# christoskokas/gtsam-vSLAM

Measured on AMD Instinct MI355X. Metric: frames/sec (extract+match+localBA), 1500 feat stereo 752x480, higher is better.
Workload: dtype u8/i32 (extract, match) + f64 (pose LM, local BA)

## Files before the change

### gtsam-vslam_amd/csrc/extract_kernels.hip

```cpp
#include "extract_kernels.hpp"
#include "../../include/vslam_orb_pattern.h"
#include <cfloat>

namespace vslam {

__constant__ __attribute__((aligned(16))) signed char c_pattern[1024];

void upload_pattern() {
    (void)hipMemcpyToSymbol(HIP_SYMBOL(c_pattern), VSLAM_ORB_PATTERN, 1024);
}

__device__ __forceinline__ int resize_hsum(unsigned d0, unsigned d1, unsigned d2, bool upper, unsigned sel, int coef) {
    typedef short s16x2 __attribute__((ext_vector_type(2)));
    const unsigned taps = __builtin_amdgcn_perm(upper ? d2 : d1, upper ? d1 : d0, sel);
    return __builtin_amdgcn_sdot2(__builtin_bit_cast(s16x2, taps), __builtin_bit_cast(s16x2, coef), 0, false);
}

__global__ __launch_bounds__(256) void k_resize(uint8_t* __restrict__ pyr, PyrDesc P, int level,
                                                const int2* __restrict__ xtab,
                                                const int2* __restrict__ ytab) {
    const int img = blockIdx.z;
    const uint8_t* __restrict__ S = pyr + (size_t)img * P.imgStride + P.off[level - 1];
    uint8_t* __restrict__ D = pyr + (size_t)img * P.imgStride + P.off[level];
    const int sp = P.pitch[level - 1], dp = P.pitch[level];
    const int dw = P.w[level], dh = P.h[level], sh = P.h[level - 1];
    const int x0 = (blockIdx.x * 64 + threadIdx.x) * 4;
    const int y = blockIdx.y * 4 + __builtin_amdgcn_readfirstlane(threadIdx.y);
    if (y >= dh || x0 >= dw) return;
    const int2 yt = ytab[y];
    int sy0 = yt.x, sy1 = yt.x + 1;
    sy0 = sy0 < 0 ? 0 : (sy0 < sh ? sy0 : sh - 1);
    sy1 = sy1 < 0 ? 0 : (sy1 < sh ? sy1 : sh - 1);
    const int b0 = (short)(yt.y & 0xffff), b1 = (short)(yt.y >> 16);
    const uint8_t* r0 = S + (size_t)sy0 * sp;
    const uint8_t* r1 = S + (size_t)sy1 * sp;
    const int4 ta = *(const int4*)(xtab + x0), tb = *(const int4*)(xtab + x0 + 2);
    const int xs[4] = {ta.x, ta.z, tb.x, tb.z}, xc[4] = {ta.y, ta.w, tb.y, tb.w};
    const int base = (xs[0] & 0xffff) & ~3;
    int o0[4], o1[4];
    bool fits = true;
#pragma unroll
    for (int i = 0; i < 4; i++) {
        o0[i] = (xs[i] & 0xffff) - base;
        o1[i] = (int)((unsigned)xs[i] >> 16) - base;
        fits = fits && (unsigned)o0[i] < 12u && (unsigned)o1[i] < 12u && (unsigned)(o1[i] - o0[i]) <= 1u;
    }
    unsigned o = 0;
    if (fits) {
        const unsigned a0 = *(const unsigned*)(r0 + base), a1 = *(const unsigned*)(r0 + base + 4), a2 = *(const unsigned*)(r0 + base + 8);
        const unsigned c0 = *(const unsigned*)(r1 + base), c1 = *(const unsigned*)(r1 + base + 4), c2 = *(const unsigned*)(r1 + base + 8);
#pragma unroll
        for (int i = 0; i < 4; i++) {
            const bool upper = o1[i] > 7 || o0[i] > 7;
            const int sh4 = upper ? 4 : 0;
            const unsigned sel = (unsigned)(o0[i] - sh4) | ((unsigned)(o1[i] - sh4) << 16) | 0x0c000c00u;
            const int h0 = resize_hsum(a0, a1, a2, upper, sel, xc[i]);
            const int h1 = resize_hsum(c0, c1, c2, upper, sel, xc[i]);
            const unsigned v = (unsigned)((((b0 * (h0 >> 4)) >> 16) + ((b1 * (h1 >> 4)) >> 16) + 2) >> 2) & 0xffu;
            o |= (x0 + i < dw ? v : 0u) << (8 * i);
        }
    } else {
        uint8_t* op = (uint8_t*)&o;
#pragma unroll
        for (int i = 0; i < 4; i++) {
            if (x0 + i < dw) {
                const int sx = xs[i] & 0xffff, sx1 = (int)((unsigned)xs[i] >> 16);
                const int c0 = (short)(xc[i] & 0xffff), c1 = (short)(xc[i] >> 16);
                const int h0 = r0[sx] * c0 + r0[sx1] * c1;
                const int h1 = r1[sx] * c0 + r1[sx1] * c1;
                op[i] = (uint8_t)((((b0 * (h0 >> 4)) >> 16) + ((b1 * (h1 >> 4)) >> 16) + 2) >> 2);
            }
        }
    }
    *(unsigned*)(D + (size_t)y * dp + x0) = o;
}

__global__ __launch_bounds__(256) void k_load_images(const uint8_t* const* __restrict__ src, int stride, uint8_t* __restrict__ pyr,
                                                     PyrDesc P) {
    const int img = blockIdx.z;
    const uint8_t* __restrict__ S = src[img];
    if (!S) return;
    uint8_t* __restrict__ D = pyr + (size_t)img * P.imgStride + P.off[0];
    const int w = P.w[0], h = P.h[0], dp = P.pitch[0];
    const int y = blockIdx.y * 4 + threadIdx.y;
    const int x0 = (blockIdx.x * 64 + threadIdx.x) * 16;
    if (y >= h || x0 >= w) return;
    const uint8_t* sp = S + (size_t)y * stride + x0;
    uint8_t* dq = D + (size_t)y * dp + x0;
    if (x0 + 16 <= w && ((((uintptr_t)sp) | ((uintptr_t)dq)) & 15) == 0) *(uint4*)dq = *(const uint4*)sp;
    else for (int i = 0; i < 16 && x0 + i < w; i++) dq[i] = sp[i];
}
void launch_load_images(hipStream_t s, const uint8_t* const* dSrc, int stride, uint8_t* pyr, const PyrDesc& P, int nimg) {
    hipLaunchKernelGGL(k_load_images, dim3((P.w[0] + 1023) / 1024, (P.h[0] + 3) / 4, nimg), dim3(64, 4), 0, s, dSrc, stride, pyr, P);
}

template <int CN>
__global__ __launch_bounds__(256) void k_load_images_color(const uint8_t* const* __restrict__ src, int stride,
                                                           uint8_t* __restrict__ pyr, PyrDesc P) {
    const int img = blockIdx.z;
    const uint8_t* __restrict__ S = src[img];
    if (!S) return;
    uint8_t* __restrict__ D = pyr + (size_t)img * P.imgStride + P.off[0];
    const int w = P.w[0], h = P.h[0], dp = P.pitch[0];
    const int y = blockIdx.y * 4 + threadIdx.y;
    const int x0 = (blockIdx.x * 64 + threadIdx.x) * 16;
    if (y >= h || x0 >= w) return;
    const uint8_t* sp = S + (size_t)y * stride + (size_t)x0 * CN;
    uint8_t* dq = D + (size_t)y * dp + x0;
    if (x0 + 16 <= w && ((((uintptr_t)sp) | ((uintptr_t)dq)) & 15) == 0) {
        unsigned wd[4 * CN];
#pragma unroll
        for (int k = 0; k < CN; k++) {
            const uint4 v = ((const uint4*)sp)[k];
            wd[4 * k] = v.x; wd[4 * k + 1] = v.y; wd[4 * k + 2] = v.z; wd[4 * k + 3] = v.w;
        }
        unsigned o[4] = {0u, 0u, 0u, 0u};
#pragma unroll
        for (int p = 0; p < 16; p++) {
            const int bi = p * CN;
            const int b = (wd[bi >> 2] >> (8 * (bi & 3))) & 0xff;
            const int g = (wd[(bi + 1) >> 2] >> (8 * ((bi + 1) & 3))) & 0xff;
            const int r = (wd[(bi + 2) >> 2] >> (8 * ((bi + 2) & 3))) & 0xff;
            o[p >> 2] |= (unsigned)bgr_to_gray(b, g, r) << (8 * (p & 3));
        }
        *(uint4*)dq = make_uint4(o[0], o[1], o[2], o[3]);
    } else {
        for (int i = 0; i < 16 && x0 + i < w; i++)
            dq[i] = (uint8_t)bgr_to_gray(sp[i * CN], sp[i * CN + 1], sp[i * CN + 2]);
    }
}
void launch_load_images_color(hipStream_t s, const uint8_t* const* dSrc, int stride, int channels, uint8_t* pyr, const PyrDesc& P,
                              int nimg) {
    const dim3 grid((P.w[0] + 1023) / 1024, (P.h[0] + 3) / 4, nimg), block(64, 4);
    if (channels == 3) hipLaunchKernelGGL(k_load_images_color<3>, grid, block, 0, s, dSrc, stride, pyr, P);
    else hipLaunchKernelGGL(k_load_images_color<4>, grid, block, 0, s, dSrc, stride, pyr, P);
}

#define VS_GLOBAL __attribute__((address_space(1)))
typedef const VS_GLOBAL uint8_t* gbytes_t;
struct __attribute__((packed)) Packed2 { unsigned short v; };
struct __attribute__((packed)) Packed4 { unsigned v; };
// ... 447 lines not shown
                 uint32_t* cellSlots, int* cellCount, int maxThr, int minThr, int nimg) {
    dim3 grid((F.cellBase[P.nLevels] + 3) / 4, xcd_image_rows(nimg));
    const size_t lds = (size_t)4 * ((size_t)F.tileRows * F.tilePitch * 2 + 2 * (FQ_MASK + 1) * 2 + FQ3_CAP * 2);
    int listCap = FQ3_CAP;
    if (const char* e = getenv("VSLAM_FAST_LIST_CAP")) listCap = std::max(0, std::min(FQ3_CAP, atoi(e)));
    hipLaunchKernelGGL(k_fast, grid, dim3(256), lds, s, pyr, P, F, cellSlots, cellCount, maxThr, minThr, listCap, nimg);
}

#ifdef VSLAM_FAST_CHECK
int fast_check_failures(hipStream_t s) {
    int n = 0;
    if (hipStreamSynchronize(s) != hipSuccess) return -1;
    if (hipMemcpyFromSymbol(&n, HIP_SYMBOL(g_fastCheckFail), sizeof(int)) != hipSuccess) return -1;
    return n;
}
#endif

__global__ __launch_bounds__(1024) void k_gather(const uint32_t* __restrict__ cellSlots,
                                                 const int* __restrict__ cellCount, FastDesc F,
                                                 int nLevels, int* __restrict__ cellOff,
                                                 uint32_t* __restrict__ cand, int candCap,
                                                 int* __restrict__ levelCount) {
    extern __shared__ int soff[];
    __shared__ int wtot[16];
    __shared__ int s_run;
    const int img = blockIdx.x, tid = threadIdx.x, lane = tid & 63, wave = tid >> 6;
    const int nCells = F.cellBase[nLevels];
    const int* cnt = cellCount + (size_t)img * nCells;
    if (tid == 0) s_run = 0;
    __syncthreads();
    for (int base = 0; base < nCells; base += 1024) {
        const int i = base + tid;
        const int v = i < nCells ? cnt[i] : 0;
        int incl = v;
#pragma unroll
        for (int d = 1; d < 64; d <<= 1) {
            const int n = __shfl_up(incl, d);
            if (lane >= d) incl += n;
        }
        if (lane == 63) wtot[wave] = incl;
        __syncthreads();
        int woff = 0;
        for (int k = 0; k < wave; k++) woff += wtot[k];
        const int run = s_run;
        if (i < nCells) soff[i] = run + woff + incl - v;
        __syncthreads();
        if (tid == 1023) s_run = run + woff + incl;
        __syncthreads();
    }
    const int total = s_run;
    if (tid == 0) soff[nCells] = total;
    __syncthreads();
    if (blockIdx.y == 0) {
        int* off = cellOff + (size_t)img * (nCells + 1);
        for (int i = tid; i <= nCells; i += 1024) off[i] = soff[i];
        if (tid < nLevels) levelCount[img * (MAX_LEVELS + 1) + tid] = soff[F.cellBase[tid + 1]] - soff[F.cellBase[tid]];
        if (tid == 0) levelCount[img * (MAX_LEVELS + 1) + MAX_LEVELS] = total;
    }
    uint32_t* out = cand + (size_t)img * candCap;
    const int lim = min(total, candCap);
    for (int j = blockIdx.y * 1024 + tid; j < lim; j += gridDim.y * 1024) {
        int lo = 0, hi = nCells;
        while (lo < hi) {
            const int mid = (lo + hi) >> 1;
            if (soff[mid + 1] > j) hi = mid; else lo = mid + 1;
        }
        out[j] = cellSlots[((size_t)img * nCells + lo) * F.cellCap + (j - soff[lo])];
    }
}

void launch_gather(hipStream_t s, const uint32_t* cellSlots, const int* cellCount, const FastDesc& F,
                   int nLevels, int* cellOff, uint32_t* cand, int candCap, int* levelCount, int nimg) {
    const int nCells = F.cellBase[nLevels];
    hipLaunchKernelGGL(k_gather, dim3(nimg, 8), dim3(1024), (size_t)(nCells + 1) * sizeof(int), s, cellSlots, cellCount, F, nLevels,
                       cellOff, cand, candCap, levelCount);
}

__device__ __forceinline__ int reflect101(int p, int len) {
    if (len == 1) return 0;
    while (p < 0 || p >= len) p = p < 0 ? -p : 2 * len - 2 - p;
    return p;
}

__global__ __launch_bounds__(256) void k_blur(const uint8_t* __restrict__ pyr,
                                              uint8_t* __restrict__ blur, PyrDesc P, BlurDesc B) {
    const int img = blockIdx.y;
    int level = 0;
    const int t = blockIdx.x;
    while (level + 1 < P.nLevels && t >= B.tileBase[level + 1]) level++;
    const int lt = t - B.tileBase[level];
    const int tyb = lt / B.tilesX[level], txb = lt - tyb * B.tilesX[level];
    const int w = P.w[level], h = P.h[level], pitch = P.pitch[level];
    const uint8_t* __restrict__ S = pyr + (size_t)img * P.imgStride + P.off[level];
    uint8_t* __restrict__ D = blur + (size_t)img * P.imgStride + P.off[level];
    const int x = txb * BLUR_TW + (threadIdx.x & 63) * 4;
    const int yb = tyb * BLUR_TH + __builtin_amdgcn_readfirstlane(threadIdx.x >> 6) * BLUR_RPT;
    if (yb >= h || x >= w) return;
    const unsigned tA = (unsigned)B.taps[0] | ((unsigned)B.taps[1] << 8) | ((unsigned)B.taps[2] << 16) | ((unsigned)B.taps[3] << 24);
    const unsigned tB = (unsigned)B.taps[4] | ((unsigned)B.taps[5] << 8) | ((unsigned)B.taps[6] << 16);
    const int t0 = B.taps[0], t1 = B.taps[1], t2 = B.taps[2], t3 = B.taps[3];
    const int m = w - x;
    unsigned s1 = 0x07060504u;
    unsigned sA = 0x03020100u, sB = 0x07060504u;
    if (m == 1) s1 = 0x01020304u;
    else if (m == 2) { s1 = 0x03040504u; sA = 0x00000002u; sB = 0x07060500u; }
    else if (m == 3) { s1 = 0x05060504u; sA = 0x00000304u; sB = 0x07060100u; }
    else if (m == 4) { sA = 0x00040506u; sB = 0x07020100u; }
    else if (m == 5) { sA = 0x05060700u; sB = 0x03020104u; }
    else if (m == 6) sB = 0x07040504u;
    const bool leftEdge = x == 0;
    const unsigned xo0 = leftEdge ? 0u : (unsigned)(x - 4), xo1 = (unsigned)x;
    unsigned hb[7][4];
#pragma unroll
    for (int rr = 0; rr < BLUR_RPT + 6; rr++) {
        int sy = yb + rr - 3;
        sy = sy < 0 ? -sy : sy;
        sy = sy >= h ? 2 * h - 2 - sy : sy;
        sy = sy < 0 ? 0 : sy;
        const uint8_t* row = S + (size_t)sy * pitch;
        unsigned d0 = *(const unsigned*)(row + xo0);
        const uint2 d12 = *(const uint2*)(row + xo1);
        unsigned d1 = d12.x, d2 = d12.y;
        {
            const unsigned mir = __builtin_amdgcn_perm(d2, d1, 0x01020304u);
            const unsigned tmp = __builtin_amdgcn_perm(d1, d0, sA);
            const unsigned n1 = __builtin_amdgcn_perm(d1, d0, s1);
            d2 = __builtin_amdgcn_perm(d2, tmp, sB);
            d1 = n1;
            d0 = leftEdge ? mir : d0;
        }
        unsigned nh[4];
        nh[0] = __builtin_amdgcn_udot4(__builtin_amdgcn_alignbyte(d1, d0, 1), tA, __builtin_amdgcn_udot4(__builtin_amdgcn_alignbyte(d2, d1, 1), tB, 0u, false), false);
        nh[1] = __builtin_amdgcn_udot4(__builtin_amdgcn_alignbyte(d1, d0, 2), tA, __builtin_amdgcn_udot4(__builtin_amdgcn_alignbyte(d2, d1, 2), tB, 0u, false), false);
        nh[2] = __builtin_amdgcn_udot4(__builtin_amdgcn_alignbyte(d1, d0, 3), tA, __builtin_amdgcn_udot4(__builtin_amdgcn_alignbyte(d2, d1, 3), tB, 0u, false), false);
        nh[3] = __builtin_amdgcn_udot4(d1, tA, __builtin_amdgcn_udot4(d2, tB, 0u, false), false);
#pragma unroll
        for (int i = 0; i < 4; i++) {
#pragma unroll
            for (int k = 0; k < 6; k++) hb[k][i] = hb[k + 1][i];
            hb[6][i] = nh[i] & 0xffffu;
        }
        if (rr >= 6) {
            const int y = yb + rr - 6;
            if (y < h) {
                unsigned o = 0;
#pragma unroll
                for (int i = 0; i < 4; i++) {
                    const unsigned acc = (unsigned)t0 * (hb[0][i] + hb[6][i]) + (unsigned)t1 * (hb[1][i] + hb[5][i]) +
                                         (unsigned)t2 * (hb[2][i] + hb[4][i]) + (unsigned)t3 * hb[3][i];
                    o |= ((acc + 32768u) >> 16) << (8 * i);
                }
                uint8_t* dq = D + (size_t)y * pitch + x;
                if (x + 4 <= w) *(unsigned*)dq = o;
                else for (int i = 0; i < 4 && x + i < w; i++) dq[i] = (uint8_t)(o >> (8 * i));
            }
        }
    }
}

void launch_blur(hipStream_t s, const uint8_t* pyr, uint8_t* blur, const PyrDesc& P,
                 const BlurDesc& B, int nimg) {
    hipLaunchKernelGGL(k_blur, dim3(B.tileBase[P.nLevels], nimg), dim3(256), 0, s, pyr, blur, P, B);
}

__device__ __forceinline__ float fast_atan2_deg(float y, float x) {
    const float scale = (float)(180 / 3.1415926535897932384626433832795);
    const float p1 = 0.9997878412794807f * scale;
    const float p3 = -0.3258083974640975f * scale;
    const float p5 = 0.1555786518463281f * scale;
    const float p7 = -0.04432655554792128f * scale;
    const float ax = fabsf(x), ay = fabsf(y);
    float a, c, c2;
    if (ax >= ay) {
        c = ay / (ax + (float)DBL_EPSILON);
        c2 = c * c;
        a = (((p7 * c2 + p5) * c2 + p3) * c2 + p1) * c;
    } else {
        c = ax / (ay + (float)DBL_EPSILON);
        c2 = c * c;
        a = 90.f - (((p7 * c2 + p5) * c2 + p3) * c2 + p1) * c;
    }
    if (x < 0) a = 180.f - a;
    if (y < 0) a = 360.f - a;
    return a;
}

__device__ __forceinline__ void sincos_deg_range(float xf, float& s_out, float& c_out) {
    const double x = (double)xf;
    const double kd = rint(x * 6.36619772367581382433e-01);
    const int k = (int)kd;
    double r = fma(-kd, 1.57079632673412561417e+00, x);
    r = fma(-kd, 6.07710050650619224932e-11, r);
    const double z = r * r;
    double ps = fma(z, 1.58969099521155010221e-10, -2.50507602534068634195e-08);
    ps = fma(z, ps, 2.75573137070700676789e-06);
    ps = fma(z, ps, -1.98412698298579493134e-04);
    ps = fma(z, ps, 8.33333333332248946124e-03);
    const double sn = fma(z * r, fma(z, ps, -1.66666666666666324348e-01), r);
    double pc = fma(z, -1.13596475577881948265e-11, 2.08757232129817482790e-09);
    pc = fma(z, pc, -2.75573143513906633035e-07);
    pc = fma(z, pc, 2.48015872894767294178e-05);
    pc = fma(z, pc, -1.38888888888741095749e-03);
    pc = fma(z, pc, 4.16666666666666019037e-02);
    const double cs = 1.0 - fma(0.5, z, -(z * (z * pc)));
    const double sq = (k & 1) ? cs : sn, cq = (k & 1) ? sn : cs;
    s_out = (float)((k & 2) ? -sq : sq);
    c_out = (float)(((k + 1) & 2) ? -cq : cq);
}

constexpr int OD_MROWS = 31, OD_MDW = 9;
constexpr int OD_ROWS = 39, OD_DW = 11;
__global__ __launch_bounds__(256) void k_orient_desc(
    const uint8_t* __restrict__ pyr, const uint8_t* __restrict__ blur, PyrDesc P, LevelTables T,
    const uint32_t* __restrict__ kept, const int* __restrict__ keptOff, int keptCap,
    DiscRows R, vslam_keypoint* __restrict__ kps,
    uint8_t* __restrict__ desc, int outCap, int nimg) {
    const int lane = threadIdx.x & 63;
    const int wave = __builtin_amdgcn_readfirstlane(threadIdx.x >> 6);
    int chunk, img;
    if (!xcd_image_block(nimg, chunk, img)) return;
    const int g = chunk * 4 + wave;
    const int* koff = keptOff + img * (MAX_LEVELS + 1);
    const int total = koff[P.nLevels];
    if (g >= total || g >= outCap) return;
    const int4 pat4 = *(const int4*)(c_pattern + 16 * lane);
    int level = 0;
    while (level + 1 < P.nLevels && g >= koff[level + 1]) level++;
    const uint32_t pk = kept[(size_t)img * keptCap + g];
    const int x = cand_x(pk), y = cand_y(pk), score = cand_s(pk);
    const int pitch = P.pitch[level];
    const size_t lvlOff = (size_t)img * P.imgStride + P.off[level];
    __shared__ unsigned sDisc[4][OD_MROWS * OD_MDW];
    __shared__ unsigned sPatch[4][OD_ROWS * OD_DW];
    unsigned* patch = sPatch[wave];
    const int xa = (x - 19) & ~3, xoff = (x - 19) - xa;
    int m10, m01 = 0;
    {
        unsigned* disc = sDisc[wave];
        const int xm = (x - 15) & ~3, xmo = (x - 15) - xm;
        const uint8_t* __restrict__ msrc = pyr + lvlOff + (size_t)(y - 15) * pitch + xm;
        unsigned w5[5];
#pragma unroll
        for (int k = 0; k < 5; k++) {
            const int i = k * 64 + lane, r = (i * 7282) >> 16, c = i - r * OD_MDW;
            w5[k] = i < OD_MROWS * OD_MDW ? *(const unsigned*)(msrc + (size_t)r * pitch + 4 * c) : 0u;
        }
        {
            const uint8_t* __restrict__ bsrc = blur + lvlOff + (size_t)(y - 19) * pitch + xa;
            unsigned v[7];
#pragma unroll
            for (int k = 0; k < 7; k++) {
                const int i = k * 64 + lane, r = (i * 5958) >> 16, c = i - r * OD_DW;
                v[k] = i < OD_ROWS * OD_DW ? *(const unsigned*)(bsrc + (size_t)r * pitch + 4 * c) : 0u;
            }
#pragma unroll
            for (int k = 0; k < 5; k++) { const int i = k * 64 + lane; if (i < OD_MROWS * OD_MDW) disc[i] = w5[k]; }
#pragma unroll
            for (int k = 0; k < 7; k++) { const int i = k * 64 + lane; if (i < OD_ROWS * OD_DW) patch[i] = v[k]; }
        }
        asm volatile("s_waitcnt vmcnt(0) lgkmcnt(0)" ::: "memory");
        const uint8_t* mb = (const uint8_t*)disc + xmo;
        const unsigned lu = lane & 31;
        const int u = (int)lu - 15, au = u < 0 ? -u : u;
        const bool neg = lane >= 32;
        const unsigned centre = 15u * (unsigned)(OD_MDW * 4) + 15u;
        const unsigned step = neg ? 0u - (unsigned)(OD_MDW * 4) : (unsigned)(OD_MDW * 4);
        unsigned off = 15u * (unsigned)(OD_MDW * 4) + lu;
        int I[16];
        bool act[16];
#pragma unroll
        for (int v = 0; v < 16; v++) {
            act[v] = au <= R.umax[v] && lu != 31u && !(neg && v == 0);
            I[v] = mb[act[v] ? off : centre];
            off += step;
        }
        int colSum = 0;
#pragma unroll
        for (int v = 0; v < 16; v++) {
            const int Iv = act[v] ? I[v] : 0;
            colSum += Iv;
            m01 += v * Iv;
        }
        m10 = u * colSum;
        if (neg) m01 = -m01;
    }
#pragma unroll
    for (int d = 32; d >= 1; d >>= 1) {
        m10 += __shfl_xor(m10, d);
        m01 += __shfl_xor(m01, d);
    }
    const float angle = fast_atan2_deg((float)m01, (float)m10);

    const float factorPI = (float)(3.1415926535897932384626433832795 / 180.f);
    const float ang = angle * factorPI;
    float a, b;
    sincos_deg_range(ang, b, a);
    const uint8_t* pb = (const uint8_t*)patch + 19 * (OD_DW * 4) + 19 + xoff;
    const int pw[4] = {pat4.x, pat4.y, pat4.z, pat4.w};
    int nib = 0;
#pragma unroll
    for (int j = 0; j < 4; j++) {
        const float x0 = (float)(signed char)(pw[j] & 0xff), y0 = (float)(signed char)((pw[j] >> 8) & 0xff);
        const float x1 = (float)(signed char)((pw[j] >> 16) & 0xff), y1 = (float)(pw[j] >> 24);
        const int ry0 = __float2int_rn(x0 * b + y0 * a), rx0 = __float2int_rn(x0 * a - y0 * b);
        const int ry1 = __float2int_rn(x1 * b + y1 * a), rx1 = __float2int_rn(x1 * a - y1 * b);
        const int t0 = pb[ry0 * (OD_DW * 4) + rx0];
        const int t1 = pb[ry1 * (OD_DW * 4) + rx1];
        nib |= (t0 < t1) << j;
    }
    const int other = __shfl_xor(nib, 1);
    const size_t o = (size_t)img * outCap + g;
    if ((lane & 1) == 0) desc[o * 32 + (lane >> 1)] = (uint8_t)(nib | (other << 4));
    if (lane == 0) {
        vslam_keypoint k;
        const float sc = T.scalePyr[level];
        k.x = (float)x;
        k.y = (float)y;
        if (level != 0) { k.x *= sc; k.y *= sc; }
        k.size = (float)T.scaledPatch[level];
        k.angle = angle;
        k.response = (float)score;
        k.octave = level;
        k.class_id = -1;
        kps[o] = k;
    }
}

void launch_orient_desc(hipStream_t s, const uint8_t* pyr, const uint8_t* blur, const PyrDesc& P,
                        const LevelTables& T, const uint32_t* kept, const int* keptOff, int keptCap,
                        const DiscRows& disc, vslam_keypoint* kps, uint8_t* desc, int outCap,
                        int maxKept, int nimg) {
    if (maxKept <= 0) return;
    hipLaunchKernelGGL(k_orient_desc, dim3((maxKept + 3) / 4, xcd_image_rows(nimg)), dim3(256), 0, s, pyr, blur, P, T,
                       kept, keptOff, keptCap, disc, kps, desc, outCap, nimg);
}

}
```

### gtsam-vslam_amd/csrc/extract_kernels.hpp

```cpp
#pragma once
#include "common.hpp"

namespace vslam {

struct PyrDesc {
    int nLevels;
    int w[MAX_LEVELS], h[MAX_LEVELS], pitch[MAX_LEVELS];
    uint32_t off[MAX_LEVELS];
    uint32_t imgStride;
};

struct FastDesc {
    int minXY;
    int edge3;
    int nCols[MAX_LEVELS], nRows[MAX_LEVELS], gridW[MAX_LEVELS], gridH[MAX_LEVELS];
    int cellBase[MAX_LEVELS + 1];
    int cellCap;
    int tileRows, tilePitch;
};

struct BlurDesc {
    int tilesX[MAX_LEVELS];
    int tileBase[MAX_LEVELS + 1];
    int taps[7];
};

struct LevelTables {
    float scalePyr[MAX_LEVELS];
    int scaledPatch[MAX_LEVELS];
};

__host__ __device__ static inline uint32_t pack_cand(int x, int y, int s) {
    return ((uint32_t)y << 20) | ((uint32_t)x << 8) | (uint32_t)s;
}
__host__ __device__ static inline int cand_x(uint32_t p) { return (p >> 8) & 0xfff; }
__host__ __device__ static inline int cand_y(uint32_t p) { return p >> 20; }
__host__ __device__ static inline int cand_s(uint32_t p) { return p & 0xff; }

constexpr int FAST_TILE_PITCH = 80;
constexpr int FAST_TILE_MAX = 76;
constexpr int BLUR_RPT = 16;
constexpr int BLUR_TW = 256, BLUR_TH = 4 * BLUR_RPT;

void launch_load_images(hipStream_t s, const uint8_t* const* dSrc, int stride, uint8_t* pyr, const PyrDesc& P, int nimg);
void launch_load_images_color(hipStream_t s, const uint8_t* const* dSrc, int stride, int channels, uint8_t* pyr, const PyrDesc& P,
                              int nimg);
struct RectSrc {
    const uint8_t* src; const float* mapX; const float* mapY;
    int sw, sh, stride, pad;
};
void launch_load_images_rect(hipStream_t s, const RectSrc* dTab, int channels, uint8_t* pyr, const PyrDesc& P, int nimg);
void launch_resize(hipStream_t s, uint8_t* pyr, const PyrDesc& P, int level, const int2* xtab,
                   const int2* ytab, int nimg);
void launch_fast(hipStream_t s, const uint8_t* pyr, const PyrDesc& P, const FastDesc& F,
                 uint32_t* cellSlots, int* cellCount, int maxThr, int minThr, int nimg);
#ifdef VSLAM_FAST_CHECK
int fast_check_failures(hipStream_t s);
#endif
void launch_gather(hipStream_t s, const uint32_t* cellSlots, const int* cellCount, const FastDesc& F,
                   int nLevels, int* cellOff, uint32_t* cand, int candCap, int* levelCount, int nimg);
void launch_blur(hipStream_t s, const uint8_t* pyr, uint8_t* blur, const PyrDesc& P,
                 const BlurDesc& B, int nimg);
struct DiscRows { int umax[16]; };
void launch_orient_desc(hipStream_t s, const uint8_t* pyr, const uint8_t* blur, const PyrDesc& P,
                        const LevelTables& T, const uint32_t* kept, const int* keptOff, int keptCap,
                        const DiscRows& disc, vslam_keypoint* kps, uint8_t* desc, int outCap,
                        int maxKept, int nimg);
void upload_pattern();

constexpr int SSC_NMAX_LDS = 16384;
constexpr int SSC_NMAX = 65535;
constexpr int SSC_PICKW_G = 2048;
struct SscArgs {
    const uint32_t* cand; int candCap; const int* levelCount;
    int nLevels, nimg;
    int numRet[MAX_LEVELS], cols[MAX_LEVELS], rows[MAX_LEVELS], high[MAX_LEVELS], kmin[MAX_LEVELS], kmax[MAX_LEVELS];
    uint32_t* tmp;
    uint32_t* gridG;
    const size_t* gridOff;
    uint32_t* aG; uint32_t* sortedG; uint32_t* picksG;
    int forceGlobal;
    int* taskCount;
    int* flags;
};

void launch_ssc(hipStream_t s, const SscArgs& A, uint32_t* kept, int keptCap, int* keptOff, int* hostCounts);

}
```

### gtsam-vslam_amd/csrc/extractor.hip

```cpp
#include "extractor.hpp"
#include <atomic>
#include <algorithm>
#include <cmath>
#include <mutex>

namespace vslam {

static thread_local char g_err[512] = "";
void set_error(const char* fmt, ...) {
    va_list ap;
    va_start(ap, fmt);
    vsnprintf(g_err, sizeof(g_err), fmt, ap);
    va_end(ap);
}

}

using namespace vslam;

static void build_fe_tables(vslam_extractor& e) {
    const int nL = e.nLevels;
    const vslam_fe_params& p = e.prm;
    e.scalePyramid.assign(nL, 1.f);
    e.scaleInvPyramid.assign(nL, 1.f);
// ... 106 lines not shown
        T.scalePyr[l] = scalePyramid[l];
        T.scaledPatch[l] = scaledPatchSize[l];
    }
    P.imgStride = (uint32_t)off;

    F.minXY = p->edge_threshold - 3;
    F.edge3 = p->edge_threshold - 3;
    int cells = 0, cap = 1, tRows = 8, tCols = 8;
    for (int l = 0; l < nLevels; l++) {
        const int maxX = P.w[l] - F.edge3, maxY = P.h[l] - F.edge3;
        const int wid = maxX - F.minXY, hig = maxY - F.minXY;
        const int nC = (int)((float)wid / 35.f), nR = (int)((float)hig / 35.f);
        if (nC < 1 || nR < 1) { set_error("pyramid level %d too small for the FAST grid", l); return VSLAM_ERR_INVALID; }
        F.nCols[l] = nC; F.nRows[l] = nR;
        F.gridW[l] = cv_ceil_f((float)wid / nC);
        F.gridH[l] = cv_ceil_f((float)hig / nR);
        if (F.gridW[l] + 6 > FAST_TILE_MAX || F.gridH[l] + 6 > FAST_TILE_MAX) {
            set_error("FAST cell larger than the LDS tile"); return VSLAM_ERR_INVALID;
        }
        F.cellBase[l] = cells;
        cells += nC * nR;
        cap = std::max(cap, ((F.gridW[l] + 1) / 2) * ((F.gridH[l] + 1) / 2));
        tRows = std::max(tRows, F.gridH[l] + 6); tCols = std::max(tCols, F.gridW[l] + 6);
    }
    F.tileRows = tRows;
    F.tilePitch = align_up(tCols + 3, 4);
    F.cellBase[nLevels] = cells;
    for (int l = nLevels + 1; l <= MAX_LEVELS; l++) F.cellBase[l] = cells;
    F.cellCap = cap;
    nCells = cells;

    int tiles = 0;
    for (int l = 0; l < nLevels; l++) {
        B.tilesX[l] = (P.w[l] + BLUR_TW - 1) / BLUR_TW;
        B.tileBase[l] = tiles;
        tiles += B.tilesX[l] * ((P.h[l] + BLUR_TH - 1) / BLUR_TH);
    }
    B.tileBase[nLevels] = tiles;
    build_gauss_taps(B.taps);

    VS_HIP(vslam::create_main_stream(&stream));
    VS_HIP(hipEventCreateWithFlags(&evGather, hipEventDisableTiming));
    VS_HIP(hipEventCreateWithFlags(&evDone, hipEventDisableTiming));
    timer.stream = stream;
    VS_HIP(hipMalloc(&d_pyr, (size_t)nimg * P.imgStride + 256));
    VS_HIP(hipMalloc(&d_blur, (size_t)nimg * P.imgStride + 256));
    VS_HIP(vslam::memset_sync(d_pyr, 0, (size_t)nimg * P.imgStride));
    VS_HIP(vslam::memset_sync(d_blur, 0, (size_t)nimg * P.imgStride));

    std::vector<int2> allx, ally;
    xtabOff.assign(nLevels, 0);
    ytabOff.assign(nLevels, 0);
    for (int l = 1; l < nLevels; l++) {
        std::vector<int2> xt, yt;
        build_resize_tables(P.w[l - 1], P.h[l - 1], P.w[l], P.h[l], xt, yt);
        while (xt.size() % 4) xt.push_back(xt.back());
        xtabOff[l] = (int)allx.size();
        ytabOff[l] = (int)ally.size();
        allx.insert(allx.end(), xt.begin(), xt.end());
        ally.insert(ally.end(), yt.begin(), yt.end());
    }
    if (allx.empty()) { allx.push_back(make_int2(0, 0)); ally.push_back(make_int2(0, 0)); }
    VS_HIP(hipMalloc(&d_xtab, allx.size() * sizeof(int2)));
    VS_HIP(hipMalloc(&d_ytab, ally.size() * sizeof(int2)));
    VS_HIP(hipMemcpy(d_xtab, allx.data(), allx.size() * sizeof(int2), hipMemcpyHostToDevice));
    VS_HIP(hipMemcpy(d_ytab, ally.data(), ally.size() * sizeof(int2), hipMemcpyHostToDevice));

    VS_HIP(hipMalloc(&d_cellSlots, (size_t)nimg * nCells * F.cellCap * sizeof(uint32_t)));
    VS_HIP(hipMalloc(&d_cellCount, (size_t)nimg * nCells * sizeof(int)));
    VS_HIP(hipMalloc(&d_cellOff, (size_t)nimg * (nCells + 1) * sizeof(int)));
    candCap = nCells * F.cellCap;
    VS_HIP(hipMalloc(&d_cand, (size_t)nimg * candCap * sizeof(uint32_t)));
    VS_HIP(hipMalloc(&d_levelCount, (size_t)nimg * (MAX_LEVELS + 1) * sizeof(int)));

    keptCap = 0;
    for (int l = 0; l < nLevels; l++) keptCap += (int)std::ceil(featurePerLevel[l] * 1.1f) + 2;
    keptCap = align_up(keptCap, 64);
    VS_HIP(hipMalloc(&d_kept, (size_t)nimg * keptCap * sizeof(uint32_t)));
    VS_HIP(hipMalloc(&d_keptOff, (size_t)nimg * (MAX_LEVELS + 1) * sizeof(int)));
    VS_HIP(hipMalloc(&d_kps, (size_t)nimg * keptCap * sizeof(vslam_keypoint)));
    VS_HIP(hipMalloc(&d_desc, (size_t)nimg * keptCap * 32));

    for (int v = 0; v < 16; v++) discRows.umax[v] = umax[v];
    nKept.assign(nimg, 0);
    for (int l = 0; l < nLevels; l++) {
        const int numRet = featurePerLevel[l], cols = P.w[l], rows = P.h[l];
        const int e1 = rows + cols + 2 * numRet;
        const long long e2 = 4LL * cols + 4LL * numRet + 4LL * rows * numRet + (long long)rows * rows +
                             (long long)cols * cols - 2LL * rows * cols + 4LL * rows * cols * numRet;
        const double e3 = std::sqrt((double)e2), e4 = numRet - 1;
        const double s1 = -std::round((e1 + e3) / e4), s2 = -std::round((e1 - e3) / e4);
        sscHigh[l] = (int)(s1 > s2 ? s1 : s2);
        const unsigned K = (unsigned)numRet;
        sscKmin[l] = (int)(unsigned)std::round((float)K - ((float)K * 0.1f));
        sscKmax[l] = (int)(unsigned)std::round((float)K + ((float)K * 0.1f));
    }
    VS_HIP(hipMalloc(&d_sscTmp, (size_t)3 * nimg * candCap * sizeof(uint32_t)));
    VS_HIP(hipMalloc(&d_sscPicks, (size_t)nimg * nLevels * 8 * SSC_PICKW_G * sizeof(uint32_t)));
    {
        size_t words = 0;
        std::vector<size_t> off((size_t)nimg * nLevels, 0);
        for (int i = 0; i < nimg; i++)
            for (int l = 0; l < nLevels; l++) {
                off[(size_t)i * nLevels + l] = words;
                words += (size_t)(2 * P.h[l] + 2) * (size_t)((2 * P.w[l] + 2 + 31) / 32);
            }
        VS_HIP(hipMalloc(&d_sscGrid, words * sizeof(uint32_t)));
        VS_HIP(hipMalloc(&d_sscGridOff, off.size() * sizeof(size_t)));
        VS_HIP(hipMemcpy(d_sscGridOff, off.data(), off.size() * sizeof(size_t), hipMemcpyHostToDevice));
    }
    VS_HIP(hipMalloc(&d_taskCount, (size_t)nimg * MAX_LEVELS * sizeof(int) + (size_t)nimg * MAX_LEVELS * 8 * sizeof(long long)));
    VS_HIP(hipMalloc(&d_sscFlags, (size_t)nimg * 2 * sizeof(int)));
    VS_HIP(vslam::memset_sync(d_sscFlags, 0, (size_t)nimg * 2 * sizeof(int)));
    VS_HIP(hipHostMalloc(&h_counts, (size_t)nimg * 3 * sizeof(int), hipHostMallocMapped));
    VS_HIP(hipHostGetDevicePointer((void**)&d_counts, h_counts, 0));
    memset(h_counts, 0, (size_t)nimg * 3 * sizeof(int));
    if (const char* e = getenv("VSLAM_SSC_FORCE_GLOBAL")) sscForceGlobal = atoi(e) != 0;
    return VSLAM_OK;
}

void vslam_extractor::release() {
    if (stream) hipStreamSynchronize(stream);
    timer.destroy();
    hipFree(d_pyr); hipFree(d_blur); hipFree(d_xtab); hipFree(d_ytab);
    hipFree(d_cellSlots); hipFree(d_cellCount); hipFree(d_cellOff);
    hipFree(d_cand); hipFree(d_levelCount);
    if (doubleOut) { hipFree(d_kpsBuf[0]); hipFree(d_kpsBuf[1]); hipFree(d_descBuf[0]); hipFree(d_descBuf[1]); }
    else { hipFree(d_kps); hipFree(d_desc); }
    hipFree(d_kept); hipFree(d_keptOff);
    hipFree(d_sscTmp); hipFree(d_sscPicks); hipFree(d_taskCount); hipFree(d_sscFlags); hipFree(d_sscGrid); hipFree(d_sscGridOff);
    d_sscGrid = nullptr; d_sscGridOff = nullptr; d_sscPicks = nullptr;
    if (h_counts) hipHostFree(h_counts);
    if (h_imgPtrs) hipHostFree(h_imgPtrs);
    hipFree(d_imgPtrs); h_imgPtrs = nullptr; d_imgPtrs = nullptr;
    if (h_colPtrs) hipHostFree(h_colPtrs);
    hipFree(d_colPtrs); hipFree(d_colStage); h_colPtrs = nullptr; d_colPtrs = nullptr; d_colStage = nullptr; colStageBytes = 0;
    if (evColPtrs) hipEventDestroy(evColPtrs);
    evColPtrs = nullptr;
    if (h_rectTab) hipHostFree(h_rectTab);
    hipFree(d_rectTab); h_rectTab = nullptr; d_rectTab = nullptr;
    if (evRectTab) hipEventDestroy(evRectTab);
    evRectTab = nullptr;
    d_sscTmp = nullptr; d_taskCount = nullptr; d_sscFlags = nullptr; h_counts = nullptr;
    if (evGather) hipEventDestroy(evGather);
    if (evDone) hipEventDestroy(evDone);
    evGather = evDone = nullptr;
    if (stream) hipStreamDestroy(stream);
    stream = nullptr;
}

void vslam_extractor::add_consumer(hipEvent_t e) {
    std::lock_guard<std::mutex> lk(consumersMu);
    for (hipEvent_t c : consumers) if (c == e) return;
    consumers.push_back(e);
}
void vslam_extractor::remove_consumer(hipEvent_t e) {
    std::lock_guard<std::mutex> lk(consumersMu);
    consumers.erase(std::remove(consumers.begin(), consumers.end(), e), consumers.end());
}
void vslam_extractor::wait_consumers() {
    std::lock_guard<std::mutex> lk(consumersMu);
    for (hipEvent_t c : consumers) hipStreamWaitEvent(stream, c, 0);
}

vslam_status vslam_extractor::set_image(int idx, const void* src, int stride, bool srcOnDevice) {
    if (idx < 0 || idx >= nimg || !src || stride < width) { set_error("set_image: bad argument"); return VSLAM_ERR_INVALID; }
// ... 141 lines not shown

vslam_status vslam_extractor::wait_counts() {
    if (!countsPending) return VSLAM_OK;
    VS_HIP(hipSetDevice(device));
    VS_HIP(hipEventSynchronize(evDone));
    countsPending = false;
#ifdef VSLAM_SSC_STAMPS
    {
        std::vector<long long> st((size_t)nimg * nLevels * 8);
        hipMemcpy(st.data(), d_taskCount + nimg * MAX_LEVELS, st.size() * sizeof(long long), hipMemcpyDeviceToHost);
        for (int i = 0; i < nimg; i++) for (int l = 0; l < nLevels; l++) { const long long* q = &st[(size_t)(i * nLevels + l) * 8]; fprintf(stderr, "ssc img %d lvl %d: n %lld partitions %lld countsort %lld search %lld (probes %lld final w %lld) emit %lld\n", i, l, q[4], q[0], q[1], q[2], q[5], q[6], q[3]); }
    }
#endif
    for (int i = 0; i < nimg; i++) {
        if (h_counts[nimg + 2 * i + 1]) { set_error("FAST candidate / kept-keypoint overflow"); return VSLAM_ERR_CAPACITY; }
        if (h_counts[nimg + 2 * i]) {
            set_error("SSC: image %d exceeds a kernel limit (mask %d: 1 = more than %d candidates in one level, 4 = segment list, "
                      "8 / 32 = width search, 16 = probe grid)", i, h_counts[nimg + 2 * i], SSC_NMAX);
            return VSLAM_ERR_CAPACITY;
        }
        nKept[i] = h_counts[i];
    }
    return VSLAM_OK;
}

vslam_status vslam_extractor::enqueue_ssc() {
    SscArgs S{};
    S.cand = d_cand; S.candCap = candCap; S.levelCount = d_levelCount; S.nLevels = nLevels; S.nimg = nimg;
    for (int l = 0; l < nLevels; l++) {
        S.numRet[l] = featurePerLevel[l]; S.cols[l] = P.w[l]; S.rows[l] = P.h[l];
        S.high[l] = sscHigh[l]; S.kmin[l] = sscKmin[l]; S.kmax[l] = sscKmax[l];
    }
    S.gridG = d_sscGrid; S.gridOff = d_sscGridOff;
    S.tmp = d_sscTmp; S.aG = d_sscTmp + (size_t)nimg * candCap; S.sortedG = d_sscTmp + (size_t)2 * nimg * candCap;
    S.picksG = d_sscPicks; S.forceGlobal = sscForceGlobal ? 1 : 0;
    S.taskCount = d_taskCount; S.flags = d_sscFlags;
    launch_ssc(stream, S, d_kept, keptCap, d_keptOff, d_counts);
    return VSLAM_OK;
}

#ifdef VSLAM_HOST_STAMPS
#include <chrono>
static double hs_now() { return std::chrono::duration<double, std::micro>(std::chrono::steady_clock::now().time_since_epoch()).count(); }
#define HS(k) hs[k] = hs_now()
#else
#define HS(k) do {} while (0)
#endif

vslam_status vslam_extractor::run() {
    VS_HIP(hipSetDevice(device));
    int t;
#ifdef VSLAM_HOST_STAMPS
    double hs[8];
#endif
    HS(0);
    wait_consumers();
    t = timer.begin("pyramid");
    for (int l = 1; l < nLevels; l++)
        launch_resize(stream, d_pyr, P, l, d_xtab + xtabOff[l], d_ytab + ytabOff[l], nimg);
    timer.end(t);
    t = timer.begin("fast");
    launch_fast(stream, d_pyr, P, F, d_cellSlots, d_cellCount, prm.max_fast_threshold,
                prm.min_fast_threshold, nimg);
    timer.end(t);
#ifdef VSLAM_FAST_CHECK
    if (const int bad = fast_check_failures(stream)) {
        set_error("k_fast: %d pixels on which a packed stage disagrees with its scalar form", bad);
        return VSLAM_ERR_HIP;
    }
#endif
    t = timer.begin("gather");
    launch_gather(stream, d_cellSlots, d_cellCount, F, nLevels, d_cellOff, d_cand, candCap,
                  d_levelCount, nimg);
    timer.end(t);
    VS_HIP(hipEventRecord(evGather, stream));
    t = timer.begin("ssc");
    VS_CHECK(enqueue_ssc());
    timer.end(t);
    t = timer.begin("blur");
    launch_blur(stream, d_pyr, d_blur, P, B, nimg);
    timer.end(t);
    t = timer.begin("orient_desc");
    if (doubleOut) { outSel ^= 1; d_kps = d_kpsBuf[outSel]; d_desc = d_descBuf[outSel]; }
    launch_orient_desc(stream, d_pyr, d_blur, P, T, d_kept, d_keptOff, keptCap, discRows, d_kps,
                       d_desc, keptCap, keptCap, nimg);
    timer.end(t);
    VS_HIP(hipGetLastError());
    VS_HIP(hipEventRecord(evDone, stream));
    countsPending = true;
    ran = true;
    return VSLAM_OK;
}

static std::atomic<int> g_poison{-2};
int vslam::poison_byte() {
    int v = g_poison.load(std::memory_order_relaxed);
    if (v == -2) {
        const char* e = getenv("VSLAM_POISON");
        v = e ? ((int)strtol(e, nullptr, 0) & 0xff) : -1;
        g_poison.store(v);
    }
    return v;
}

extern "C" {

void vslam_thread_release(void) { vslam::thread_release(); }

vslam_status vslam_device_alloc(int32_t device, size_t bytes, void** out) {
    if (!out || !bytes) return VSLAM_ERR_INVALID;
    VS_HIP(hipSetDevice(device));
    VS_HIP(hipMalloc(out, bytes));
    return VSLAM_OK;
}
vslam_status vslam_device_upload(int32_t device, void* dst, const void* src, size_t bytes) {
    if (!dst || !src) return VSLAM_ERR_INVALID;
    VS_HIP(hipSetDevice(device));
    VS_HIP(hipMemcpy(dst, src, bytes, hipMemcpyHostToDevice));
    return VSLAM_OK;
}
vslam_status vslam_device_download(int32_t device, void* dst, const void* src, size_t bytes) {
    if (!dst || !src) return VSLAM_ERR_INVALID;
    VS_HIP(hipSetDevice(device));
    VS_HIP(hipMemcpy(dst, src, bytes, hipMemcpyDeviceToHost));
    return VSLAM_OK;
}
void vslam_device_free(int32_t device, void* p) {
    if (p && hipSetDevice(device) == hipSuccess) hipFree(p);
}

void vslam_debug_poison(int32_t byte) { g_poison.store(byte < 0 ? -1 : (byte & 0xff)); }

const char* vslam_last_error(void) { return vslam::g_err; }

int vslam_device_count(void) {
    int n = 0;
    if (hipGetDeviceCount(&n) != hipSuccess) return 0;
    return n;
}

vslam_status vslam_extractor_create(const vslam_fe_params* params, int32_t width, int32_t height,
                                    int32_t batch, int32_t device, vslam_extractor** out) {
    if (!out) return VSLAM_ERR_INVALID;
    *out = nullptr;
    vslam_extractor* e = new (std::nothrow) vslam_extractor();
    if (!e) return VSLAM_ERR_INVALID;
    vslam_status s = e->init(params, width, height, batch, device);
    if (s != VSLAM_OK) { e->release(); delete e; return s; }
    *out = e;
    return VSLAM_OK;
}

void vslam_extractor_destroy(vslam_extractor* ex) {
    if (!ex) return;
    ex->release();
    delete ex;
}

vslam_status vslam_extractor_tables(const vslam_extractor* ex, float* sp, float* si, float* sg,
                                    float* isg, int32_t* ps, int32_t* fpl) {
    if (!ex) return VSLAM_ERR_INVALID;
    for (int i = 0; i < ex->nLevels; i++) {
        if (sp) sp[i] = ex->scalePyramid[i];
        if (si) si[i] = ex->scaleInvPyramid[i];
        if (sg) sg[i] = ex->sigmaFactor[i];
        if (isg) isg[i] = ex->InvSigmaFactor[i];
        if (ps) ps[i] = ex->scaledPatchSize[i];
// ... 173 lines not shown
```

Baseline: 30480.

## Vectorize orientation moments with disc tables and packed-dot blur

Replaces the per-lane scalar column walk for the intensity-centroid moments with precomputed per-row disc mask/weight tables in constant memory. Each lane now handles one disc row with udot4 byte dot products, and the reduction uses DPP. The vertical blur pass packs row pairs into 16-bit halves and accumulates with udot2, and the edge store becomes a masked word write. Smaller tweaks use mul24, a branchless atan, and clamped loads in place of predicated patch loads. The masked full-word blur store near the right edge could write past the row width into pitch padding.

```diff
diff --git a/gtsam-vslam_amd/csrc/disc_tables.hpp b/gtsam-vslam_amd/csrc/disc_tables.hpp
--- /dev/null
+++ b/gtsam-vslam_amd/csrc/disc_tables.hpp
@@ -0,0 +1,24 @@
+#pragma once
+#include <cstdint>
+
+namespace vslam {
+
+constexpr int DISC_HALF = 15;
+constexpr int DISC_ROW_DW = 8;
+constexpr int DISC_TAB_DW = 20;
+constexpr int DISC_TAB_ENTRIES = DISC_HALF + 1;
+
+inline void build_disc_tables(const int umax[DISC_HALF + 1], uint32_t out[DISC_TAB_ENTRIES * DISC_TAB_DW]) {
+    for (int av = 0; av <= DISC_HALF; av++) {
+        uint32_t* e = out + av * DISC_TAB_DW;
+        for (int c = 0; c < DISC_TAB_DW; c++) e[c] = 0;
+        for (int b = 0; b <= 2 * DISC_HALF; b++) {
+            const int u = b - DISC_HALF;
+            if (u < -umax[av] || u > umax[av]) continue;
+            e[b >> 2] |= 1u << (8 * (b & 3));
+            e[DISC_ROW_DW + (b >> 2)] |= (uint32_t)b << (8 * (b & 3));
+        }
+    }
+}
+
+}
diff --git a/gtsam-vslam_amd/csrc/extract_kernels.hip b/gtsam-vslam_amd/csrc/extract_kernels.hip
--- a/gtsam-vslam_amd/csrc/extract_kernels.hip
+++ b/gtsam-vslam_amd/csrc/extract_kernels.hip
@@ -1,4 +1,5 @@
 #include "extract_kernels.hpp"
+#include "disc_tables.hpp"
 #include "../../include/vslam_orb_pattern.h"
 #include <cfloat>
 
@@ -8,6 +9,14 @@
 
 void upload_pattern() {
     (void)hipMemcpyToSymbol(HIP_SYMBOL(c_pattern), VSLAM_ORB_PATTERN, 1024);
+}
+
+__constant__ __attribute__((aligned(16))) uint32_t c_discTab[DISC_TAB_ENTRIES * DISC_TAB_DW];
+
+hipError_t upload_disc_tables(const DiscRows& disc) {
+    uint32_t tab[DISC_TAB_ENTRIES * DISC_TAB_DW];
+    build_disc_tables(disc.umax, tab);
+    return hipMemcpyToSymbol(HIP_SYMBOL(c_discTab), tab, sizeof(tab));
 }
 
 __device__ __forceinline__ int resize_hsum(unsigned d0, unsigned d1, unsigned d2, bool upper, unsigned sel, int coef) {
@@ -56,7 +65,7 @@
             const unsigned sel = (unsigned)(o0[i] - sh4) | ((unsigned)(o1[i] - sh4) << 16) | 0x0c000c00u;
             const int h0 = resize_hsum(a0, a1, a2, upper, sel, xc[i]);
             const int h1 = resize_hsum(c0, c1, c2, upper, sel, xc[i]);
-            const unsigned v = (unsigned)((((b0 * (h0 >> 4)) >> 16) + ((b1 * (h1 >> 4)) >> 16) + 2) >> 2) & 0xffu;
+            const unsigned v = (unsigned)(((__mul24(b0, h0 >> 4) >> 16) + (__mul24(b1, h1 >> 4) >> 16) + 2) >> 2) & 0xffu;
             o |= (x0 + i < dw ? v : 0u) << (8 * i);
         }
     } else {
@@ -670,6 +679,11 @@
     return p;
 }
 
+__device__ __forceinline__ unsigned blur_dot2(unsigned rows, unsigned taps, unsigned acc) {
+    typedef unsigned short u16x2 __attribute__((ext_vector_type(2)));
+    return __builtin_amdgcn_udot2(__builtin_bit_cast(u16x2, rows), __builtin_bit_cast(u16x2, taps), acc, false);
+}
+
 __global__ __launch_bounds__(256) void k_blur(const uint8_t* __restrict__ pyr,
                                               uint8_t* __restrict__ blur, PyrDesc P, BlurDesc B) {
     const int img = blockIdx.y;
@@ -686,7 +700,9 @@
     if (yb >= h || x >= w) return;
     const unsigned tA = (unsigned)B.taps[0] | ((unsigned)B.taps[1] << 8) | ((unsigned)B.taps[2] << 16) | ((unsigned)B.taps[3] << 24);
     const unsigned tB = (unsigned)B.taps[4] | ((unsigned)B.taps[5] << 8) | ((unsigned)B.taps[6] << 16);
-    const int t0 = B.taps[0], t1 = B.taps[1], t2 = B.taps[2], t3 = B.taps[3];
+    const unsigned c0x = (unsigned)B.taps[0] & 0xffu, c12 = ((unsigned)B.taps[1] & 0xffu) | (((unsigned)B.taps[2] & 0xffu) << 16);
+    const unsigned c34 = ((unsigned)B.taps[3] & 0xffu) | (((unsigned)B.taps[4] & 0xffu) << 16);
+    const unsigned c56 = ((unsigned)B.taps[5] & 0xffu) | (((unsigned)B.taps[6] & 0xffu) << 16);
     const int m = w - x;
     unsigned s1 = 0x07060504u;
     unsigned sA = 0x03020100u, sB = 0x07060504u;
@@ -696,9 +712,16 @@
     else if (m == 4) { sA = 0x00040506u; sB = 0x07020100u; }
     else if (m == 5) { sA = 0x05060700u; sB = 0x03020104u; }
     else if (m == 6) sB = 0x07040504u;
+    const unsigned omask = m >= 4 ? 0xffffffffu : (1u << (8 * m)) - 1u;
     const bool leftEdge = x == 0;
     const unsigned xo0 = leftEdge ? 0u : (unsigned)(x - 4), xo1 = (unsigned)x;
-    unsigned hb[7][4];
+    unsigned pr[6][4], hp[4];
+#pragma unroll
+    for (int i = 0; i < 4; i++) {
+        hp[i] = 0;
+#pragma unroll
+        for (int j = 0; j < 6; j++) pr[j][i] = 0;
+    }
 #pragma unroll
     for (int rr = 0; rr < BLUR_RPT + 6; rr++) {
         int sy = yb + rr - 3;
@@ -706,8 +729,10 @@
         sy = sy >= h ? 2 * h - 2 - sy : sy;
         sy = sy < 0 ? 0 : sy;
         const uint8_t* row = S + (size_t)sy * pitch;
-        unsigned d0 = *(const unsigned*)(row + xo0);
-        const uint2 d12 = *(const uint2*)(row + xo1);
+        unsigned o0 = xo0, o1 = xo1;
+        asm volatile("" : "+v"(o0), "+v"(o1));
+        unsigned d0 = *(const unsigned*)(row + o0);
+        const uint2 d12 = *(const uint2*)(row + o1);
         unsigned d1 = d12.x, d2 = d12.y;
         {
             const unsigned mir = __builtin_amdgcn_perm(d2, d1, 0x01020304u);
@@ -725,22 +750,25 @@
 #pragma unroll
         for (int i = 0; i < 4; i++) {
 #pragma unroll
-            for (int k = 0; k < 6; k++) hb[k][i] = hb[k + 1][i];
-            hb[6][i] = nh[i] & 0xffffu;
+            for (int k = 0; k < 5; k++) pr[k][i] = pr[k + 1][i];
+            pr[5][i] = hp[i] | (nh[i] << 16);
+            hp[i] = nh[i];
         }
         if (rr >= 6) {
             const int y = yb + rr - 6;
             if (y < h) {
-                unsigned o = 0;
+                unsigned acc[4];
 #pragma unroll
                 for (int i = 0; i < 4; i++) {
-                    const unsigned acc = (unsigned)t0 * (hb[0][i] + hb[6][i]) + (unsigned)t1 * (hb[1][i] + hb[5][i]) +
-                                         (unsigned)t2 * (hb[2][i] + hb[4][i]) + (unsigned)t3 * hb[3][i];
-                    o |= ((acc + 32768u) >> 16) << (8 * i);
+                    acc[i] = blur_dot2(pr[0][i], c0x, 32768u);
+                    acc[i] = blur_dot2(pr[1][i], c12, acc[i]);
+                    acc[i] = blur_dot2(pr[3][i], c34, acc[i]);
+                    acc[i] = blur_dot2(pr[5][i], c56, acc[i]);
                 }
-                uint8_t* dq = D + (size_t)y * pitch + x;
-                if (x + 4 <= w) *(unsigned*)dq = o;
-                else for (int i = 0; i < 4 && x + i < w; i++) dq[i] = (uint8_t)(o >> (8 * i));
+                const unsigned o = __builtin_amdgcn_perm(acc[1], acc[0], 0x0c0c0602u) |
+                                   (__builtin_amdgcn_perm(acc[3], acc[2], 0x0c0c0602u) << 16);
+                uint8_t* drow = D + (size_t)y * pitch;
+                *(unsigned*)(drow + o1) = o & omask;
             }
         }
     }
@@ -758,16 +786,11 @@
     const float p5 = 0.1555786518463281f * scale;
     const float p7 = -0.04432655554792128f * scale;
     const float ax = fabsf(x), ay = fabsf(y);
-    float a, c, c2;
-    if (ax >= ay) {
-        c = ay / (ax + (float)DBL_EPSILON);
-        c2 = c * c;
-        a = (((p7 * c2 + p5) * c2 + p3) * c2 + p1) * c;
-    } else {
-        c = ax / (ay + (float)DBL_EPSILON);
-        c2 = c * c;
-        a = 90.f - (((p7 * c2 + p5) * c2 + p3) * c2 + p1) * c;
-    }
+    const bool xmaj = ax >= ay;
+    const float c = (xmaj ? ay : ax) / ((xmaj ? ax : ay) + (float)DBL_EPSILON);
+    const float c2 = c * c;
+    const float p = (((p7 * c2 + p5) * c2 + p3) * c2 + p1) * c;
+    float a = xmaj ? p : 90.f - p;
     if (x < 0) a = 180.f - a;
     if (y < 0) a = 360.f - a;
     return a;
@@ -796,12 +819,24 @@
     c_out = (float)(((k + 1) & 2) ? -cq : cq);
 }
 
+__device__ __forceinline__ int wave_sum32(int v) {
+    v += __builtin_amdgcn_update_dpp(0, v, 0xB1, 0xf, 0xf, true);
+    v += __builtin_amdgcn_update_dpp(0, v, 0x4E, 0xf, 0xf, true);
+    v += __builtin_amdgcn_update_dpp(0, v, 0x141, 0xf, 0xf, true);
+    v += __builtin_amdgcn_update_dpp(0, v, 0x140, 0xf, 0xf, true);
+    return __builtin_amdgcn_readlane(v, 0) + __builtin_amdgcn_readlane(v, 16);
+}
+
+static_assert(DISC_ROW_DW == 8 && DISC_HALF == 15 && DISC_TAB_ENTRIES * DISC_TAB_DW == 5 * 64,
+              "the disc tables are laid out for the 31-column row and copied by a wave in five loads");
 constexpr int OD_MROWS = 31, OD_MDW = 9;
 constexpr int OD_ROWS = 39, OD_DW = 11;
+constexpr int OD_PATCH_DW = (OD_ROWS * OD_DW + 3) & ~3;
+static_assert(DISC_TAB_ENTRIES * DISC_TAB_DW <= OD_PATCH_DW, "the disc's row vectors borrow the descriptor patch's LDS");
 __global__ __launch_bounds__(256) void k_orient_desc(
     const uint8_t* __restrict__ pyr, const uint8_t* __restrict__ blur, PyrDesc P, LevelTables T,
     const uint32_t* __restrict__ kept, const int* __restrict__ keptOff, int keptCap,
-    DiscRows R, vslam_keypoint* __restrict__ kps,
+    vslam_keypoint* __restrict__ kps,
     uint8_t* __restrict__ desc, int outCap, int nimg) {
     const int lane = threadIdx.x & 63;
     const int wave = __builtin_amdgcn_readfirstlane(threadIdx.x >> 6);
@@ -819,10 +854,12 @@
     const int pitch = P.pitch[level];
     const size_t lvlOff = (size_t)img * P.imgStride + P.off[level];
     __shared__ unsigned sDisc[4][OD_MROWS * OD_MDW];
-    __shared__ unsigned sPatch[4][OD_ROWS * OD_DW];
+    __shared__ __attribute__((aligned(16))) unsigned sPatch[4][OD_PATCH_DW];
     unsigned* patch = sPatch[wave];
+    unsigned* sTab = patch;
     const int xa = (x - 19) & ~3, xoff = (x - 19) - xa;
-    int m10, m01 = 0;
+    int m10, m01;
+    unsigned pv[7];
     {
         unsigned* disc = sDisc[wave];
         const int xm = (x - 15) & ~3, xmo = (x - 15) - xm;
@@ -830,53 +867,48 @@
         unsigned w5[5];
 #pragma unroll
         for (int k = 0; k < 5; k++) {
-            const int i = k * 64 + lane, r = (i * 7282) >> 16, c = i - r * OD_MDW;
-            w5[k] = i < OD_MROWS * OD_MDW ? *(const unsigned*)(msrc + (size_t)r * pitch + 4 * c) : 0u;
-        }
-        {
-            const uint8_t* __restrict__ bsrc = blur + lvlOff + (size_t)(y - 19) * pitch + xa;
-            unsigned v[7];
-#pragma unroll
-            for (int k = 0; k < 7; k++) {
-                const int i = k * 64 + lane, r = (i * 5958) >> 16, c = i - r * OD_DW;
-                v[k] = i < OD_ROWS * OD_DW ? *(const unsigned*)(bsrc + (size_t)r * pitch + 4 * c) : 0u;
-            }
-#pragma unroll
-            for (int k = 0; k < 5; k++) { const int i = k * 64 + lane; if (i < OD_MROWS * OD_MDW) disc[i] = w5[k]; }
-#pragma unroll
-            for (int k = 0; k < 7; k++) { const int i = k * 64 + lane; if (i < OD_ROWS * OD_DW) patch[i] = v[k]; }
-        }
+            const unsigned i = min(k * 64 + lane, OD_MROWS * OD_MDW - 1), r = __umul24(i, 7282u) >> 16;
+            w5[k] = *(const unsigned*)(msrc + (__umul24(r, (unsigned)(pitch - 4 * OD_MDW)) + 4 * i));
+        }
+        const uint8_t* __restrict__ bsrc = blur + lvlOff + (size_t)(y - 19) * pitch + xa;
+#pragma unroll
+        for (int k = 0; k < 7; k++) {
+            const unsigned i = min(k * 64 + lane, OD_ROWS * OD_DW - 1), r = __umul24(i, 5958u) >> 16;
+            pv[k] = *(const unsigned*)(bsrc + (__umul24(r, (unsigned)(pitch - 4 * OD_DW)) + 4 * i));
+        }
+        unsigned tv[5];
+#pragma unroll
+        for (int k = 0; k < 5; k++) tv[k] = c_discTab[k * 64 + lane];
+#pragma unroll
+        for (int k = 0; k < 5; k++) sTab[k * 64 + lane] = tv[k];
+#pragma unroll
+        for (int k = 0; k < 5; k++) { const int i = k * 64 + lane; if (i < OD_MROWS * OD_MDW) disc[i] = w5[k]; }
         asm volatile("s_waitcnt vmcnt(0) lgkmcnt(0)" ::: "memory");
-        const uint8_t* mb = (const uint8_t*)disc + xmo;
-        const unsigned lu = lane & 31;
-        const int u = (int)lu - 15, au = u < 0 ? -u : u;
-        const bool neg = lane >= 32;
-        const unsigned centre = 15u * (unsigned)(OD_MDW * 4) + 15u;
-        const unsigned step = neg ? 0u - (unsigned)(OD_MDW * 4) : (unsigned)(OD_MDW * 4);
-        unsigned off = 15u * (unsigned)(OD_MDW * 4) + lu;
-        int I[16];
-        bool act[16];
-#pragma unroll
-        for (int v = 0; v < 16; v++) {
-            act[v] = au <= R.umax[v] && lu != 31u && !(neg && v == 0);
-            I[v] = mb[act[v] ? off : centre];
-            off += step;
-        }
-        int colSum = 0;
-#pragma unroll
-        for (int v = 0; v < 16; v++) {
-            const int Iv = act[v] ? I[v] : 0;
-            colSum += Iv;
-            m01 += v * Iv;
-        }
-        m10 = u * colSum;
-        if (neg) m01 = -m01;
-    }
-#pragma unroll
-    for (int d = 32; d >= 1; d >>= 1) {
-        m10 += __shfl_xor(m10, d);
-        m01 += __shfl_xor(m01, d);
-    }
+        const int row = lane < OD_MROWS ? lane : OD_MROWS - 1;
+        const int vr = row - DISC_HALF, av = vr < 0 ? -vr : vr;
+        const uint4* tq = (const uint4*)(sTab + av * DISC_TAB_DW);
+        const uint4 q0 = tq[0], q1 = tq[1], q2 = tq[2], q3 = tq[3];
+        const unsigned mk[DISC_ROW_DW] = {q0.x, q0.y, q0.z, q0.w, q1.x, q1.y, q1.z, q1.w};
+        const unsigned wt[DISC_ROW_DW] = {q2.x, q2.y, q2.z, q2.w, q3.x, q3.y, q3.z, q3.w};
+        const unsigned* dr = disc + row * OD_MDW;
+        unsigned dw[OD_MDW];
+#pragma unroll
+        for (int c = 0; c < OD_MDW; c++) dw[c] = dr[c];
+        unsigned sI = 0, sW = 0;
+#pragma unroll
+        for (int c = 0; c < DISC_ROW_DW; c++) {
+            const unsigned d = __builtin_amdgcn_alignbyte(dw[c + 1], dw[c], (unsigned)xmo);
+            sI = __builtin_amdgcn_udot4(d, mk[c], sI, false);
+            sW = __builtin_amdgcn_udot4(d, wt[c], sW, false);
+        }
+        const int rI = lane < OD_MROWS ? (int)sI : 0, rW = lane < OD_MROWS ? (int)sW : 0;
+        m01 = __mul24(vr, rI);
+        m10 = __mul24(rI, -DISC_HALF) + rW;
+    }
+#pragma unroll
+    for (int k = 0; k < 7; k++) { const int i = k * 64 + lane; if (i < OD_ROWS * OD_DW) patch[i] = pv[k]; }
+    m10 = wave_sum32(m10);
+    m01 = wave_sum32(m01);
     const float angle = fast_atan2_deg((float)m01, (float)m10);
 
     const float factorPI = (float)(3.1415926535897932384626433832795 / 180.f);
@@ -892,8 +924,8 @@
         const float x1 = (float)(signed char)((pw[j] >> 16) & 0xff), y1 = (float)(pw[j] >> 24);
         const int ry0 = __float2int_rn(x0 * b + y0 * a), rx0 = __float2int_rn(x0 * a - y0 * b);
         const int ry1 = __float2int_rn(x1 * b + y1 * a), rx1 = __float2int_rn(x1 * a - y1 * b);
-        const int t0 = pb[ry0 * (OD_DW * 4) + rx0];
-        const int t1 = pb[ry1 * (OD_DW * 4) + rx1];
+        const int t0 = pb[__mul24(ry0, OD_DW * 4) + rx0];
+        const int t1 = pb[__mul24(ry1, OD_DW * 4) + rx1];
         nib |= (t0 < t1) << j;
     }
     const int other = __shfl_xor(nib, 1);
@@ -916,11 +948,11 @@
 
 void launch_orient_desc(hipStream_t s, const uint8_t* pyr, const uint8_t* blur, const PyrDesc& P,
                         const LevelTables& T, const uint32_t* kept, const int* keptOff, int keptCap,
-                        const DiscRows& disc, vslam_keypoint* kps, uint8_t* desc, int outCap,
+                        vslam_keypoint* kps, uint8_t* desc, int outCap,
                         int maxKept, int nimg) {
     if (maxKept <= 0) return;
     hipLaunchKernelGGL(k_orient_desc, dim3((maxKept + 3) / 4, xcd_image_rows(nimg)), dim3(256), 0, s, pyr, blur, P, T,
-                       kept, keptOff, keptCap, disc, kps, desc, outCap, nimg);
-}
-
-}
+                       kept, keptOff, keptCap, kps, desc, outCap, nimg);
+}
+
+}
diff --git a/gtsam-vslam_amd/csrc/extract_kernels.hpp b/gtsam-vslam_amd/csrc/extract_kernels.hpp
--- a/gtsam-vslam_amd/csrc/extract_kernels.hpp
+++ b/gtsam-vslam_amd/csrc/extract_kernels.hpp
@@ -62,9 +62,10 @@
 void launch_blur(hipStream_t s, const uint8_t* pyr, uint8_t* blur, const PyrDesc& P,
                  const BlurDesc& B, int nimg);
 struct DiscRows { int umax[16]; };
+hipError_t upload_disc_tables(const DiscRows& disc);
 void launch_orient_desc(hipStream_t s, const uint8_t* pyr, const uint8_t* blur, const PyrDesc& P,
                         const LevelTables& T, const uint32_t* kept, const int* keptOff, int keptCap,
-                        const DiscRows& disc, vslam_keypoint* kps, uint8_t* desc, int outCap,
+                        vslam_keypoint* kps, uint8_t* desc, int outCap,
                         int maxKept, int nimg);
 void upload_pattern();
 
diff --git a/gtsam-vslam_amd/csrc/extractor.hip b/gtsam-vslam_amd/csrc/extractor.hip
--- a/gtsam-vslam_amd/csrc/extractor.hip
+++ b/gtsam-vslam_amd/csrc/extractor.hip
@@ -212,6 +212,7 @@
     VS_HIP(hipMalloc(&d_desc, (size_t)nimg * keptCap * 32));
 
     for (int v = 0; v < 16; v++) discRows.umax[v] = umax[v];
+    VS_HIP(upload_disc_tables(discRows));
     nKept.assign(nimg, 0);
     for (int l = 0; l < nLevels; l++) {
         const int numRet = featurePerLevel[l], cols = P.w[l], rows = P.h[l];
@@ -519,7 +520,7 @@
     timer.end(t);
     t = timer.begin("orient_desc");
     if (doubleOut) { outSel ^= 1; d_kps = d_kpsBuf[outSel]; d_desc = d_descBuf[outSel]; }
-    launch_orient_desc(stream, d_pyr, d_blur, P, T, d_kept, d_keptOff, keptCap, discRows, d_kps,
+    launch_orient_desc(stream, d_pyr, d_blur, P, T, d_kept, d_keptOff, keptCap, d_kps,
                        d_desc, keptCap, keptCap, nimg);
     timer.end(t);
     VS_HIP(hipGetLastError());
```

Result: no change. 30760, median of 6 (+0.9%).
